# declare-lab/tango

Measured on NVIDIA H100. Metric: audio_seconds_per_second, higher is better.
Workload: dtype bf16

## Files before the change

tango_b200/csrc/gemm_tc.cu:

```cuda
#include "tng_ptx.cuh"
#include "tng_internal.h"
#include <stdlib.h>

namespace tng {

constexpr int BM = 128;
constexpr int BK = 64;
constexpr int A_TILE_BYTES = BM * BK * 2;
constexpr int GEMM_THREADS = 384;
constexpr int EPI_WARPS = 8;
constexpr int ES = 4;

struct KGroupDev {
  int view, a_c0, dw, dh, b_k0, nkb;
};

struct GemmKernelParams {
  int W, H, NB;
  int bw, bh, bn;
  int tiles_w, tiles_h, tiles_n;
  int m_tiles, n_tiles;
  int Ncols;
  int n_groups, total_kiters;
  int ksplit;
// ... 301 lines not shown
    const bool col_ok = col < p.Ncols;
    float4 add4 = make_float4(0.f, 0.f, 0.f, 0.f);
    if (col_ok && sp == 0 && p.bias) add4 = __ldg(reinterpret_cast<const float4*>(p.bias + col));
#pragma unroll 1
    for (int i = 0; i < ES; ++i) {
      const int rr = wr + 4 * i + rsub;
      if (!col_ok || rr >= nvalid) continue;
      const long long row = row_base + rr;
      float4 a = *reinterpret_cast<const float4*>(st + (4 * i + rsub) * 32 + ((cg ^ ((4 * i + rsub) & 7)) << 2));
      if (sp == 0) {
        a.x += add4.x; a.y += add4.y; a.z += add4.z; a.w += add4.w;
        if (p.rowvec) {
          const float4 r4 = __ldg(reinterpret_cast<const float4*>(p.rowvec + static_cast<long long>(n0 + rr / rpi) * p.rowvec_ld + col));
          a.x += r4.x; a.y += r4.y; a.z += r4.z; a.w += r4.w;
        }
        if (p.res) {
          if (p.res_bf16) {
            const float4 r4 = load_bf16x4(reinterpret_cast<const __nv_bfloat16*>(p.res) + row * p.ldr + col);
            a.x += r4.x; a.y += r4.y; a.z += r4.z; a.w += r4.w;
          } else {
            const float4 r4 = *reinterpret_cast<const float4*>(reinterpret_cast<const float*>(p.res) + row * p.ldr + col);
            a.x += r4.x; a.y += r4.y; a.z += r4.z; a.w += r4.w;
          }
        }
      }
      a.x *= p.alpha; a.y *= p.alpha; a.z *= p.alpha; a.w *= p.alpha;
      float* op = p.out_f32 + row * p.ld_f32 + col;
      atomicAdd(op, a.x); atomicAdd(op + 1, a.y); atomicAdd(op + 2, a.z); atomicAdd(op + 3, a.w);
    }
  }
}

template <int BN, bool FULL, bool SPLIT, bool TANH>
__device__ __forceinline__ void epi_tile_geglu(const GemmKernelParams& p, float* st, const float (&acc)[BN / 2], long long r0,
                                               int nleft, int tn, int lane) {
  constexpr int HALF = BN / 2;
  const int cg = lane & 7, rsub = lane >> 3;
#pragma unroll 1
  for (int c = 0; c < HALF / 32; ++c) {
    float4 hid[ES], g[ES];
    stage_chunk<BN>(st, lane, acc, c);
#pragma unroll
    for (int i = 0; i < ES; ++i) {
      const int r = 4 * i + rsub;
      hid[i] = *reinterpret_cast<const float4*>(st + r * 32 + ((cg ^ (r & 7)) << 2));
    }
    stage_chunk<BN>(st, lane, acc, c + HALF / 32);
#pragma unroll
    for (int i = 0; i < ES; ++i) {
      const int r = 4 * i + rsub;
      g[i] = *reinterpret_cast<const float4*>(st + r * 32 + ((cg ^ (r & 7)) << 2));
    }
    const int gcol = tn * BN + 32 * c + 4 * cg;
    const int ocol = tn * HALF + 32 * c + 4 * cg;
    float4 bh = make_float4(0.f, 0.f, 0.f, 0.f), bg = bh;
    if (p.bias) {
      bh = __ldg(reinterpret_cast<const float4*>(p.bias + gcol));
      bg = __ldg(reinterpret_cast<const float4*>(p.bias + gcol + HALF));
    }
#pragma unroll
    for (int i = 0; i < ES; ++i) {
      hid[i].x = (hid[i].x + bh.x) * (TANH ? gelu_tanh_f(g[i].x + bg.x) : gelu_erf_f(g[i].x + bg.x));
      hid[i].y = (hid[i].y + bh.y) * (TANH ? gelu_tanh_f(g[i].y + bg.y) : gelu_erf_f(g[i].y + bg.y));
      hid[i].z = (hid[i].z + bh.z) * (TANH ? gelu_tanh_f(g[i].z + bg.z) : gelu_erf_f(g[i].z + bg.z));
      hid[i].w = (hid[i].w + bh.w) * (TANH ? gelu_tanh_f(g[i].w + bg.w) : gelu_erf_f(g[i].w + bg.w));
    }
    __nv_bfloat16* op = p.out_bf16 + r0 * p.ld_bf16 + ocol;
    const long long os = 4 * p.ld_bf16;
#pragma unroll
    for (int i = 0; i < ES; ++i) {
      if (!FULL && 4 * i >= nleft) continue;
      uint2 u;
      u.x = pack_bf16(hid[i].x, hid[i].y); u.y = pack_bf16(hid[i].z, hid[i].w);
      *reinterpret_cast<uint2*>(op + i * os) = u;
      if (SPLIT) {
        uint2 l;
        l.x = pack_bf16_lo(hid[i].x, hid[i].y); l.y = pack_bf16_lo(hid[i].z, hid[i].w);
        *reinterpret_cast<uint2*>(op + p.split_off + i * os) = l;
      }
    }
  }
}

__device__ __forceinline__ int tile_kiters(const GemmKernelParams& p, int tile) {
  const int sp = tile % p.ksplit;
  return (sp + 1) * p.total_kiters / p.ksplit - sp * p.total_kiters / p.ksplit;
}

template <int BN>
__global__ void __launch_bounds__(GEMM_THREADS, 1)
gemm_tc_kernel(const __grid_constant__ CUtensorMap amap0, const __grid_constant__ CUtensorMap amap1,
               const __grid_constant__ CUtensorMap amap2, const __grid_constant__ CUtensorMap amap3,
               const __grid_constant__ CUtensorMap bmap, const __grid_constant__ GemmKernelParams p) {
  using Cfg = GemmCfg<BN>;
  constexpr int STAGES = Cfg::STAGES;
  extern __shared__ __align__(1024) uint8_t smem[];
  uint8_t* sA = smem;
  uint8_t* sB = smem + STAGES * A_TILE_BYTES;
  float* sEpi = reinterpret_cast<float*>(smem + STAGES * Cfg::STAGE_BYTES);
  uint64_t* full_bar = reinterpret_cast<uint64_t*>(smem + STAGES * Cfg::STAGE_BYTES + Cfg::EPI_BYTES);
  uint64_t* empty_bar = full_bar + STAGES;

  const int tid = threadIdx.x;
  const int warp = tid >> 5;
  const int lane = tid & 31;
  const int wg = warp >> 2;

  if (tid == 0) {
    if ((smem_u32(smem) & 1023u) != 0) __trap();
    tma_prefetch_desc(&amap0);
    tma_prefetch_desc(&bmap);
    for (int s = 0; s < STAGES; ++s) {
      mbar_init(&full_bar[s], 1);
      mbar_init(&empty_bar[s], 2);
    }
    fence_mbar_init();
  }
  __syncthreads();

  const int total_tiles = p.m_tiles * p.n_tiles * p.ksplit;
  const int work0 = blockIdx.x, work_stride = gridDim.x;

  if (wg == 0) {
    setmaxnreg_dec<40>();
    if (tid == 0) {
      uint32_t n_loaded = 0;
      for (int tile = work0; tile < total_tiles; tile += work_stride) {
        const int sp = tile % p.ksplit, t2 = tile / p.ksplit;
        const int tm = t2 / p.n_tiles, tn = t2 % p.n_tiles;
        const int tw = tm % p.tiles_w;
        const int th = (tm / p.tiles_w) % p.tiles_h;
        const int tb = tm / (p.tiles_w * p.tiles_h);
        const int w0 = tw * p.bw, h0 = th * p.bh, n0 = tb * p.bn;
        const int nk = tile_kiters(p, tile);
        int k = sp * p.total_kiters / p.ksplit, gi = 0;
        while (k >= p.g[gi].nkb) { k -= p.g[gi].nkb; ++gi; }
        for (int ki = 0; ki < nk; ++ki, ++k, ++n_loaded) {
          if (k == p.g[gi].nkb) { k = 0; ++gi; }
          const int slot = static_cast<int>(n_loaded % STAGES);
          const uint32_t use = n_loaded / STAGES;
          if (use > 0) mbar_wait(&empty_bar[slot], (use - 1) & 1);
          const KGroupDev g = p.g[gi];
          const CUtensorMap* am = g.view == 0 ? &amap0 : g.view == 1 ? &amap1 : g.view == 2 ? &amap2 : &amap3;
          mbar_arrive_expect_tx(&full_bar[slot], Cfg::STAGE_BYTES);
          tma_load_4d(sA + slot * A_TILE_BYTES, am, &full_bar[slot], g.a_c0 + k * BK, w0 + g.dw, h0 + g.dh, n0);
          tma_load_2d(sB + slot * Cfg::B_TILE_BYTES, &bmap, &full_bar[slot], g.b_k0 + k * BK, tn * BN);
        }
      }
    }
    return;
  }
  setmaxnreg_inc<232>();

  const int cw = warp - 4;
  float* st = sEpi + cw * (16 * 32);
  const int rsub = lane >> 3;
  const int wr = 16 * cw;
  const uint32_t a_off = static_cast<uint32_t>(wg - 1) * (64 * 128);
  const bool release = (tid & 127) == 0;
  const int mode = (p.res ? 1 : 0) | (p.out_f32 ? 2 : 0) | (p.out_bf16 ? 4 : 0);
  const bool geglu = (p.act == TNG_ACT_GEGLU || p.act == TNG_ACT_GEGLU_TANH);
  uint32_t n_used = 0;
  float acc[BN / 2];
#pragma unroll
  for (int i = 0; i < BN / 2; ++i) acc[i] = 0.f;
  for (int tile = work0; tile < total_tiles; tile += work_stride) {
    const int sp = tile % p.ksplit, t2 = tile / p.ksplit;
    const int tm = t2 / p.n_tiles, tn = t2 % p.n_tiles;
    const int nk = tile_kiters(p, tile);
    for (int ki = 0; ki < nk; ++ki) {
      const int slot = static_cast<int>(n_used % STAGES);
      mbar_wait(&full_bar[slot], (n_used / STAGES) & 1);
      const uint64_t ad = wgmma_desc_sw128(smem_u32(sA + slot * A_TILE_BYTES) + a_off, 16, 1024);
      const uint64_t bd = wgmma_desc_sw128(smem_u32(sB + slot * Cfg::B_TILE_BYTES), 16, 1024);
      fence_regs(acc);
      wgmma_fence();
#pragma unroll
      for (int k = 0; k < BK / 16; ++k) wgmma_ss<BN>(acc, ad + 2 * k, bd + 2 * k, (ki > 0 || k > 0) ? 1u : 0u);
      wgmma_commit();
      fence_regs(acc);
      if (ki > 0) {
        wgmma_wait<1>();
        fence_regs(acc);
        mbar_arrive_if(&empty_bar[(n_used - 1) % STAGES], release);
      }
      ++n_used;
    }
    wgmma_wait<0>();
    fence_regs(acc);
    mbar_arrive_if(&empty_bar[(n_used - 1) % STAGES], release);

    const int tw = tm % p.tiles_w;
    const int th = (tm / p.tiles_w) % p.tiles_h;
    const int tb = tm / (p.tiles_w * p.tiles_h);
    const int w0 = tw * p.bw, h0 = th * p.bh, n0 = tb * p.bn;
    const long long row_base = (static_cast<long long>(n0) * p.H + h0) * p.W + w0;
    int nvalid;
    if (p.bh == 1 && p.bn == 1) nvalid = min(BM, p.W - w0);
    else if (p.bn == 1) nvalid = min(p.bh, p.H - h0) * p.bw;
    else nvalid = min(p.bn, p.NB - n0) * p.bh * p.bw;
    const int rpi = p.bw * p.bh;
    const bool full = p.fast_epi && (nvalid == BM) && ((tn + 1) * BN <= p.Ncols);
    if (p.ksplit > 1) {
      epi_tile_splitk<BN>(p, st, acc, row_base, n0, rpi, nvalid, sp, tn, lane, wr);
    } else if (geglu) {
      if constexpr (BN == 128 || BN == 256) {
        const long long gr0 = row_base + wr + rsub;
        const int nleft = nvalid - (wr + rsub);
        if (p.act == TNG_ACT_GEGLU_TANH) {
          if (p.split_off > 0) epi_tile_geglu<BN, false, true, true>(p, st, acc, gr0, nleft, tn, lane);
          else epi_tile_geglu<BN, false, false, true>(p, st, acc, gr0, nleft, tn, lane);
        } else if (p.split_off > 0) epi_tile_geglu<BN, false, true, false>(p, st, acc, gr0, nleft, tn, lane);
        else if (nvalid == BM) epi_tile_geglu<BN, true, false, false>(p, st, acc, gr0, nleft, tn, lane);
        else epi_tile_geglu<BN, false, false, false>(p, st, acc, gr0, nleft, tn, lane);
      }
    } else if (!full) {
      EpiRows R;
      R.valid = 0;
#pragma unroll
      for (int i = 0; i < ES; ++i) {
        const int rr = wr + 4 * i + rsub;
        R.img[i] = n0 + rr / rpi;
        R.row[i] = row_base + rr;
        if (rr < nvalid) R.valid |= 1u << i;
      }
      if (p.fast_epi) epi_tile_generic<BN, true>(p, st, acc, R, tn, lane);
      else epi_tile_generic<BN, false>(p, st, acc, R, tn, lane);
    } else {
      const long long r0 = row_base + wr + rsub;
      const int img0 = n0 + (wr + rsub) / rpi;
      const bool rv_uniform = (rpi % 16) == 0;
      const long long simg = p.col_stats ? (row_base + wr) / p.stats_hw : 0;
      switch (mode) {
        case 2: epi_tile_full<BN, false, true, false>(p, st, acc, r0, img0, rv_uniform, tn, lane, simg); break;
        case 3: epi_tile_full<BN, true, true, false>(p, st, acc, r0, img0, rv_uniform, tn, lane, simg); break;
        case 4: epi_tile_full<BN, false, false, true>(p, st, acc, r0, img0, rv_uniform, tn, lane, simg); break;
        case 5: epi_tile_full<BN, true, false, true>(p, st, acc, r0, img0, rv_uniform, tn, lane, simg); break;
        case 6: epi_tile_full<BN, false, true, true>(p, st, acc, r0, img0, rv_uniform, tn, lane, simg); break;
        default: epi_tile_full<BN, true, true, true>(p, st, acc, r0, img0, rv_uniform, tn, lane, simg); break;
      }
    }
  }
}

template <int BN>
static int launch_gemm(const CUtensorMap* am, const CUtensorMap& bm, const GemmKernelParams& p, cudaStream_t st) {
  using Cfg = GemmCfg<BN>;
  const int rc = set_max_dynamic_smem<gemm_tc_kernel<BN>>(Cfg::SMEM_BYTES, "gemm_tc");
  if (rc) return rc;
  const int work = p.m_tiles * p.n_tiles * p.ksplit;
  const int grid = work < num_sms() ? work : num_sms();
  gemm_tc_kernel<BN><<<grid, GEMM_THREADS, Cfg::SMEM_BYTES, st>>>(am[0], am[1], am[2], am[3], bm, p);
  return check_launch("gemm_tc");
}

static bool is_pow2(long long x) { return x > 0 && (x & (x - 1)) == 0; }

}

using namespace tng;

static int plan_gemm(const tng_gemm_desc* d, GemmKernelParams& p, int& bn_tile_out, bool& stats_after_out) {
  if (!d) return set_error(TNG_EINVAL, "null desc");
  if (d->n_aviews < 1 || d->n_aviews > TNG_MAX_AVIEWS) return set_error(TNG_EINVAL, "n_aviews=%d", d->n_aviews);
  if (d->n_groups < 1 || d->n_groups > TNG_MAX_KGROUPS) return set_error(TNG_EINVAL, "n_groups=%d", d->n_groups);
  if (d->W <= 0 || d->H <= 0 || d->NB <= 0 || d->Ncols <= 0) return set_error(TNG_EINVAL, "bad output grid");
  if ((d->ldb > 0 ? d->ldb : d->Ktot) % 8 != 0)
    return set_error(TNG_EINVAL, "B row stride must be a multiple of 8 elements (Ktot=%lld ldb=%lld)", (long long)d->Ktot, (long long)d->ldb);

  memset(&p, 0, sizeof(p));
  p.W = d->W; p.H = d->H; p.NB = d->NB;
  if (d->W >= BM || d->H == 1) {
    p.bw = BM; p.bh = 1; p.bn = 1;
  } else {
    if (!is_pow2(d->W)) return set_error(TNG_EINVAL, "W=%d < 128 must be a power of two", d->W);
    p.bw = d->W;
    const int rem = BM / p.bw;
    if (d->H >= rem) {
      p.bh = rem; p.bn = 1;
    } else {
      if (!is_pow2(d->H)) return set_error(TNG_EINVAL, "H=%d (W=%d) must be a power of two when W*H < 128", d->H, d->W);
      p.bh = d->H; p.bn = rem / p.bh;
    }
  }
  p.tiles_w = (d->W + p.bw - 1) / p.bw;
  p.tiles_h = (d->H + p.bh - 1) / p.bh;
  p.tiles_n = (d->NB + p.bn - 1) / p.bn;
  p.m_tiles = p.tiles_w * p.tiles_h * p.tiles_n;
  p.Ncols = (int)d->Ncols;

  int bn_tile = d->block_n;
  int ksplit = 1;
  if (d->act == TNG_ACT_GEGLU || d->act == TNG_ACT_GEGLU_TANH) {
    if (bn_tile == 0) bn_tile = (d->Ncols % 256 == 0) ? 256 : 128;
    if ((bn_tile != 128 && bn_tile != 256) || d->Ncols % bn_tile != 0 || !d->out_bf16 || d->out_f32 || d->res ||
        d->rowvec)
      return set_error(TNG_EINVAL, "GEGLU epilogue needs block_n 128/256 dividing Ncols, bf16 output only");
  }
  if (bn_tile == 0) {
    const long long N = d->Ncols;
    if (N <= 32) bn_tile = 32;
    else if (N <= 64) bn_tile = 64;
    else if (N % 256 == 0 && (long long)p.m_tiles * (N / 256) >= 2 * num_sms()) bn_tile = 256;
    else if (N % 160 == 0) {
      bn_tile = 160;
      if ((long long)p.m_tiles * (N / 160) * 2 <= num_sms()) {
        static int splitk = -1;
        if (splitk < 0) { const char* e = getenv("TNG_GEMM_SPLITK"); splitk = e ? atoi(e) : 1; }
        long long kit = 0;
        for (int i = 0; i < d->n_groups; ++i) kit += d->g[i].nkb;
        const bool can_split = splitk && d->out_f32 && !d->out_bf16 && !d->accumulate && d->act == TNG_ACT_NONE &&
                               d->res != d->out_f32 && kit >= 32 && d->Ncols % 4 == 0;
        if (can_split) ksplit = 2;
        else if (N % 128 == 0 && (long long)p.m_tiles * (N / 128) <= num_sms()) bn_tile = 128;
      }
    }
    else if (N % 128 == 0) bn_tile = 128;
    else if (N % 64 == 0 && N < 256) bn_tile = 64;
    else bn_tile = 128;
  }
  p.n_tiles = (int)((d->Ncols + bn_tile - 1) / bn_tile);
  p.ksplit = ksplit;

  p.n_groups = d->n_groups;
  p.total_kiters = 0;
  for (int i = 0; i < d->n_groups; ++i) {
    const tng_kgroup& g = d->g[i];
    if (g.view < 0 || g.view >= d->n_aviews || g.nkb <= 0) return set_error(TNG_EINVAL, "k-group %d invalid", i);
    if (g.b_k0 < 0 || g.b_k0 + (long long)(g.nkb - 1) * BK >= d->Ktot)
      return set_error(TNG_EINVAL, "k-group %d: K block outside B", i);
    if (g.a_c0 < 0 || g.a_c0 + (long long)(g.nkb - 1) * BK >= d->a[g.view].C)
      return set_error(TNG_EINVAL, "k-group %d: K block outside view channels", i);
    p.g[i] = KGroupDev{g.view, g.a_c0, g.dw, g.dh, g.b_k0, g.nkb};
    p.total_kiters += g.nkb;
  }
  p.bias = d->bias; p.rowvec = d->rowvec; p.rowvec_ld = d->rowvec_ld > 0 ? d->rowvec_ld : d->Ncols; p.res = d->res; p.res_bf16 = (d->res_dtype == TNG_DT_BF16);
  p.ldr = d->ldr; p.alpha = d->alpha; p.accumulate = d->accumulate;
  p.out_f32 = d->out_f32; p.ld_f32 = d->ld_f32;
  p.out_bf16 = reinterpret_cast<__nv_bfloat16*>(d->out_bf16); p.ld_bf16 = d->ld_bf16;
  p.act = d->act; p.act_param = d->act_param; p.split_off = d->split_off;
  if (!d->out_f32 && !d->out_bf16) return set_error(TNG_EINVAL, "no output");
  if (d->accumulate && !d->out_f32) return set_error(TNG_EINVAL, "accumulate needs out_f32");

  auto al16 = [](const void* q) { return (reinterpret_cast<uintptr_t>(q) & 15) == 0; };
  bool vec = true;
  if (d->bias && !al16(d->bias)) vec = false;
  if (d->rowvec && (!al16(d->rowvec) || p.rowvec_ld % 4)) vec = false;
  if (d->res) {
    if (!al16(d->res)) vec = false;
    if (p.res_bf16 ? (d->ldr % 8) : (d->ldr % 4)) vec = false;
  }
  if (d->out_f32 && (!al16(d->out_f32) || d->ld_f32 % 4)) vec = false;
  if (d->out_bf16 && (!al16(d->out_bf16) || d->ld_bf16 % 8 || d->split_off % 8)) vec = false;
  p.vec_ok = vec ? 1 : 0;
  p.fast_epi = (vec && d->Ncols % 4 == 0) ? 1 : 0;
  if ((d->act == TNG_ACT_GEGLU || d->act == TNG_ACT_GEGLU_TANH) && !vec) return set_error(TNG_EINVAL, "GEGLU epilogue needs 16-byte aligned output");
  if (d->gn_stats) {
    if (d->stats_hw <= 0 || (static_cast<long long>(d->W) * d->H * d->NB) % d->stats_hw != 0)
      return set_error(TNG_EINVAL, "gn_stats: the output rows must be whole images of stats_hw pixels");
    if (!d->out_f32 && (d->split_off > 0 || d->act != TNG_ACT_NONE))
      return set_error(TNG_EINVAL, "gn_stats without an fp32 output needs a plain bf16 output (no activation, no hi/lo split)");
  }

  const bool full_m = (p.bh == 1 && p.bn == 1) ? (d->W % BM == 0) : (p.bn == 1 ? (d->H % p.bh == 0) : (d->NB % p.bn == 0));
  if (p.ksplit > 1 && !p.fast_epi) p.ksplit = 1;
  bool stats_after = false;
  if (d->gn_stats) {
    const bool fused = full_m && (d->Ncols % bn_tile == 0) && p.fast_epi && p.ksplit == 1 && !d->accumulate &&
                       (d->stats_hw % 16 == 0) && d->act != TNG_ACT_GEGLU && d->act != TNG_ACT_GEGLU_TANH;
    if (fused) { p.col_stats = d->gn_stats; p.stats_hw = d->stats_hw; }
    else stats_after = true;
  }
  bn_tile_out = bn_tile;
  stats_after_out = stats_after;
  return TNG_OK;
}

extern "C" int tng_gemm_plan(const tng_gemm_desc* d, int32_t* block_n, int32_t* mode, int32_t* ksplit) {
  GemmKernelParams p;
  int bn_tile = 0;
  bool stats_after = false;
  const int rc = plan_gemm(d, p, bn_tile, stats_after);
  if (rc != TNG_OK) return rc;
  if (block_n) *block_n = bn_tile;
  if (mode) *mode = 1;
  if (ksplit) *ksplit = p.ksplit;
  return TNG_OK;
}

extern "C" int tng_conv_gemm(const tng_gemm_desc* d, void* stream) {
  GemmKernelParams p;
  int bn_tile = 0;
  bool stats_after = false;
  {
    const int rc = plan_gemm(d, p, bn_tile, stats_after);
    if (rc != TNG_OK) return rc;
  }
  CUtensorMap am[4];
  for (int i = 0; i < 4; ++i) {
    const tng_aview& v = d->a[i < d->n_aviews ? i : 0];
    if (v.C % 8 != 0) return set_error(TNG_EINVAL, "view %d: C=%lld must be a multiple of 8", i, (long long)v.C);
    uint64_t dims[4] = {(uint64_t)v.C, (uint64_t)v.W, (uint64_t)v.H, (uint64_t)v.NB};
    uint64_t strides[3] = {(uint64_t)v.s_w * 2, (uint64_t)v.s_h * 2, (uint64_t)v.s_n * 2};
    uint32_t box[4] = {(uint32_t)BK, (uint32_t)p.bw, (uint32_t)p.bh, (uint32_t)p.bn};
    int rc = encode_tmap_bf16(&am[i], v.ptr, 4, dims, strides, box);
    if (rc) return rc;
  }
  CUtensorMap bm;
  {
    uint64_t dims[2] = {(uint64_t)d->Ktot, (uint64_t)d->Ncols};
    uint64_t strides[1] = {(uint64_t)(d->ldb > 0 ? d->ldb : d->Ktot) * 2};
    uint32_t box[2] = {(uint32_t)BK, (uint32_t)bn_tile};
    int rc = encode_tmap_bf16(&bm, d->b, 2, dims, strides, box);
    if (rc) return rc;
  }
  cudaStream_t st = reinterpret_cast<cudaStream_t>(stream);
  if (p.ksplit > 1) {
    const size_t rows = static_cast<size_t>(d->W) * d->H * d->NB;
    cudaError_t e = cudaMemset2DAsync(d->out_f32, static_cast<size_t>(d->ld_f32) * 4, 0, static_cast<size_t>(d->Ncols) * 4, rows, st);
    if (e != cudaSuccess) return set_error(TNG_ECUDA, "cudaMemset2DAsync(split-K output): %s", cudaGetErrorString(e));
  }
  int rc;
  switch (bn_tile) {
    case 32: rc = launch_gemm<32>(am, bm, p, st); break;
    case 64: rc = launch_gemm<64>(am, bm, p, st); break;
    case 128: rc = launch_gemm<128>(am, bm, p, st); break;
    case 160: rc = launch_gemm<160>(am, bm, p, st); break;
    case 256: rc = launch_gemm<256>(am, bm, p, st); break;
    default: return set_error(TNG_EINVAL, "block_n=%d unsupported", bn_tile);
  }
  if (rc == TNG_OK && stats_after) {
    const long long rows = static_cast<long long>(d->W) * d->H * d->NB;
    if (d->out_f32) rc = launch_col_stats(d->out_f32, TNG_DT_F32, d->Ncols, d->ld_f32, rows / d->stats_hw, d->stats_hw, d->gn_stats, st);
    else rc = launch_col_stats(d->out_bf16, TNG_DT_BF16, d->Ncols, d->ld_bf16, rows / d->stats_hw, d->stats_hw, d->gn_stats, st);
  }
  return rc;
}
```

tango_b200/csrc/tng_ptx.cuh:

```cuda
#pragma once
#include <cuda_runtime.h>
#include <cuda_bf16.h>
#include <cuda.h>
#include <stdint.h>
#include <stdio.h>
#include "../../include/tango_b200.h"

namespace tng {

#ifndef TNG_SPIN_LIMIT
#define TNG_SPIN_LIMIT (1u << 28)
#endif

__device__ __forceinline__ uint32_t smem_u32(const void* p) {
  return static_cast<uint32_t>(__cvta_generic_to_shared(p));
}

__device__ __forceinline__ void mbar_init(uint64_t* bar, uint32_t count) {
  asm volatile("mbarrier.init.shared::cta.b64 [%0], %1;" ::"r"(smem_u32(bar)), "r"(count));
}
__device__ __forceinline__ void fence_mbar_init() {
  asm volatile("fence.mbarrier_init.release.cluster;" ::: "memory");
}
__device__ __forceinline__ void mbar_arrive_expect_tx(uint64_t* bar, uint32_t bytes) {
  asm volatile("mbarrier.arrive.expect_tx.shared::cta.b64 _, [%0], %1;" ::"r"(smem_u32(bar)), "r"(bytes)
               : "memory");
}
__device__ __forceinline__ void mbar_arrive(uint64_t* bar) {
  asm volatile("mbarrier.arrive.shared::cta.b64 _, [%0];" ::"r"(smem_u32(bar)) : "memory");
}
__device__ __forceinline__ void mbar_arrive_if(uint64_t* bar, bool pred) {
  asm volatile(
      "{\n\t.reg .pred p;\n\tsetp.ne.b32 p, %1, 0;\n\t@p mbarrier.arrive.shared::cta.b64 _, [%0];\n\t}"
      ::"r"(smem_u32(bar)), "r"((uint32_t)pred) : "memory");
}
template <int N>
__device__ __forceinline__ void setmaxnreg_dec() { asm volatile("setmaxnreg.dec.sync.aligned.u32 %0;" ::"n"(N)); }
template <int N>
__device__ __forceinline__ void setmaxnreg_inc() { asm volatile("setmaxnreg.inc.sync.aligned.u32 %0;" ::"n"(N)); }
__device__ __forceinline__ uint32_t mbar_try_wait(uint64_t* bar, uint32_t parity) {
  uint32_t ok;
  asm volatile(
      "{\n\t"
      ".reg .pred P;\n\t"
      "mbarrier.try_wait.parity.shared::cta.b64 P, [%1], %2;\n\t"
      "selp.u32 %0, 1, 0, P;\n\t"
      "}\n"
      : "=r"(ok)
      : "r"(smem_u32(bar)), "r"(parity)
      : "memory");
  return ok;
}
__device__ __forceinline__ void mbar_wait(uint64_t* bar, uint32_t parity) {
  uint32_t spins = 0;
  while (!mbar_try_wait(bar, parity)) {
    if (++spins > TNG_SPIN_LIMIT) __trap();
  }
}

__device__ __forceinline__ void tma_prefetch_desc(const CUtensorMap* m) {
  asm volatile("prefetch.tensormap [%0];" ::"l"(reinterpret_cast<uint64_t>(m)) : "memory");
}
__device__ __forceinline__ void tma_load_2d(void* smem, const CUtensorMap* m, uint64_t* bar, int c0, int c1) {
  asm volatile(
      "cp.async.bulk.tensor.2d.shared::cluster.global.mbarrier::complete_tx::bytes [%0], [%1, {%3, %4}], [%2];"
      ::"r"(smem_u32(smem)), "l"(reinterpret_cast<uint64_t>(m)), "r"(smem_u32(bar)), "r"(c0), "r"(c1)
      : "memory");
}
__device__ __forceinline__ void tma_load_3d(void* smem, const CUtensorMap* m, uint64_t* bar, int c0, int c1,
                                            int c2) {
  asm volatile(
      "cp.async.bulk.tensor.3d.shared::cluster.global.mbarrier::complete_tx::bytes [%0], [%1, {%3, %4, %5}], [%2];"
      ::"r"(smem_u32(smem)), "l"(reinterpret_cast<uint64_t>(m)), "r"(smem_u32(bar)), "r"(c0), "r"(c1), "r"(c2)
      : "memory");
}
__device__ __forceinline__ void tma_load_4d(void* smem, const CUtensorMap* m, uint64_t* bar, int c0, int c1,
                                            int c2, int c3) {
  asm volatile(
      "cp.async.bulk.tensor.4d.shared::cluster.global.mbarrier::complete_tx::bytes [%0], [%1, {%3, %4, %5, %6}], "
      "[%2];" ::"r"(smem_u32(smem)),
      "l"(reinterpret_cast<uint64_t>(m)), "r"(smem_u32(bar)), "r"(c0), "r"(c1), "r"(c2), "r"(c3)
      : "memory");
}

__device__ __forceinline__ void wgmma_fence() { asm volatile("wgmma.fence.sync.aligned;" ::: "memory"); }
__device__ __forceinline__ void wgmma_commit() { asm volatile("wgmma.commit_group.sync.aligned;" ::: "memory"); }
template <int N>
__device__ __forceinline__ void wgmma_wait() {
  asm volatile("wgmma.wait_group.sync.aligned %0;" ::"n"(N) : "memory");
}
template <int R>
__device__ __forceinline__ void fence_regs(float (&d)[R]) {
#pragma unroll
  for (int i = 0; i < R; ++i) asm volatile("" : "+f"(d[i])::"memory");
}

__device__ __forceinline__ uint64_t wgmma_desc_sw128(uint32_t saddr, uint32_t lbo_bytes, uint32_t sbo_bytes) {
  uint64_t d = 0;
  d |= static_cast<uint64_t>((saddr & 0x3FFFF) >> 4);
  d |= static_cast<uint64_t>((lbo_bytes >> 4) & 0x3FFF) << 16;
  d |= static_cast<uint64_t>((sbo_bytes >> 4) & 0x3FFF) << 32;
  d |= static_cast<uint64_t>(1) << 62;
  return d;
}

template <int N>
__device__ __forceinline__ void wgmma_ss(float (&d)[N / 2], uint64_t a_desc, uint64_t b_desc, uint32_t scale_d);

template <>
__device__ __forceinline__ void wgmma_ss<32>(float (&d)[16], uint64_t a_desc, uint64_t b_desc, uint32_t scale_d) {
  asm volatile(
      "{\n\t.reg .pred p;\n\tsetp.ne.b32 p, %18, 0;\n\t"
      "wgmma.mma_async.sync.aligned.m64n32k16.f32.bf16.bf16 {%0, %1, %2, %3, %4, %5, %6, %7, %8, %9, %10, %11, %12, %13, %14, %15}, %16, %17, p, 1, 1, 0, 0;\n\t}\n"
      : "+f"(d[0]), "+f"(d[1]), "+f"(d[2]), "+f"(d[3]), "+f"(d[4]), "+f"(d[5]), "+f"(d[6]), "+f"(d[7]),
        "+f"(d[8]), "+f"(d[9]), "+f"(d[10]), "+f"(d[11]), "+f"(d[12]), "+f"(d[13]), "+f"(d[14]), "+f"(d[15])
      : "l"(a_desc), "l"(b_desc), "r"(scale_d));
}

template <>
__device__ __forceinline__ void wgmma_ss<64>(float (&d)[32], uint64_t a_desc, uint64_t b_desc, uint32_t scale_d) {
  asm volatile(
      "{\n\t.reg .pred p;\n\tsetp.ne.b32 p, %34, 0;\n\t"
      "wgmma.mma_async.sync.aligned.m64n64k16.f32.bf16.bf16 {%0, %1, %2, %3, %4, %5, %6, %7, %8, %9, %10, %11, %12, %13, %14, %15, %16, %17, %18, %19, %20, %21, %22, %23, %24, %25, %26, %27, %28, %29, %30, %31}, %32, %33, p, 1, 1, 0, 0;\n\t}\n"
      : "+f"(d[0]), "+f"(d[1]), "+f"(d[2]), "+f"(d[3]), "+f"(d[4]), "+f"(d[5]), "+f"(d[6]), "+f"(d[7]),
        "+f"(d[8]), "+f"(d[9]), "+f"(d[10]), "+f"(d[11]), "+f"(d[12]), "+f"(d[13]), "+f"(d[14]), "+f"(d[15]),
        "+f"(d[16]), "+f"(d[17]), "+f"(d[18]), "+f"(d[19]), "+f"(d[20]), "+f"(d[21]), "+f"(d[22]), "+f"(d[23]),
        "+f"(d[24]), "+f"(d[25]), "+f"(d[26]), "+f"(d[27]), "+f"(d[28]), "+f"(d[29]), "+f"(d[30]), "+f"(d[31])
      : "l"(a_desc), "l"(b_desc), "r"(scale_d));
}

template <>
__device__ __forceinline__ void wgmma_ss<128>(float (&d)[64], uint64_t a_desc, uint64_t b_desc, uint32_t scale_d) {
  asm volatile(
      "{\n\t.reg .pred p;\n\tsetp.ne.b32 p, %66, 0;\n\t"
      "wgmma.mma_async.sync.aligned.m64n128k16.f32.bf16.bf16 {%0, %1, %2, %3, %4, %5, %6, %7, %8, %9, %10, %11, %12, %13, %14, %15, %16, %17, %18, %19, %20, %21, %22, %23, %24, %25, %26, %27, %28, %29, %30, %31, %32, %33, %34, %35, %36, %37, %38, %39, %40, %41, %42, %43, %44, %45, %46, %47, %48, %49, %50, %51, %52, %53, %54, %55, %56, %57, %58, %59, %60, %61, %62, %63}, %64, %65, p, 1, 1, 0, 0;\n\t}\n"
      : "+f"(d[0]), "+f"(d[1]), "+f"(d[2]), "+f"(d[3]), "+f"(d[4]), "+f"(d[5]), "+f"(d[6]), "+f"(d[7]),
        "+f"(d[8]), "+f"(d[9]), "+f"(d[10]), "+f"(d[11]), "+f"(d[12]), "+f"(d[13]), "+f"(d[14]), "+f"(d[15]),
        "+f"(d[16]), "+f"(d[17]), "+f"(d[18]), "+f"(d[19]), "+f"(d[20]), "+f"(d[21]), "+f"(d[22]), "+f"(d[23]),
        "+f"(d[24]), "+f"(d[25]), "+f"(d[26]), "+f"(d[27]), "+f"(d[28]), "+f"(d[29]), "+f"(d[30]), "+f"(d[31]),
        "+f"(d[32]), "+f"(d[33]), "+f"(d[34]), "+f"(d[35]), "+f"(d[36]), "+f"(d[37]), "+f"(d[38]), "+f"(d[39]),
        "+f"(d[40]), "+f"(d[41]), "+f"(d[42]), "+f"(d[43]), "+f"(d[44]), "+f"(d[45]), "+f"(d[46]), "+f"(d[47]),
        "+f"(d[48]), "+f"(d[49]), "+f"(d[50]), "+f"(d[51]), "+f"(d[52]), "+f"(d[53]), "+f"(d[54]), "+f"(d[55]),
        "+f"(d[56]), "+f"(d[57]), "+f"(d[58]), "+f"(d[59]), "+f"(d[60]), "+f"(d[61]), "+f"(d[62]), "+f"(d[63])
      : "l"(a_desc), "l"(b_desc), "r"(scale_d));
}

template <>
__device__ __forceinline__ void wgmma_ss<160>(float (&d)[80], uint64_t a_desc, uint64_t b_desc, uint32_t scale_d) {
  asm volatile(
// ... 188 lines not shown
```

tango_b200/lib.py:

```python
from __future__ import annotations

import ctypes as C
import os
from typing import Optional, Sequence

import torch

from . import build as _build

ACT_NONE, ACT_SILU, ACT_LRELU, ACT_GEGLU, ACT_GEGLU_TANH = 0, 1, 2, 3, 4
DT_F32, DT_BF16 = 0, 1
MAX_AVIEWS, MAX_KGROUPS = 4, 40

SYMBOLS = [
    "tng_version", "tng_last_error", "tng_launch_count", "tng_conv_gemm", "tng_attention",
    "tng_groupnorm_stats", "tng_groupnorm_apply", "tng_layernorm", "tng_cast_act", "tng_softmax_rows",
    "tng_transpose_bf16", "tng_sched_step", "tng_timestep_embedding", "tng_linear_f32", "tng_convt_gather",
    "tng_tanh_to_i16", "tng_rmsnorm", "tng_gather_rows", "tng_rel_attention", "tng_stft_frames", "tng_stft_magnitude",
    "tng_log_clamp", "tng_attention_wide", "tng_gemm_plan",
]


class TangoB200Error(RuntimeError):
    pass
# ... 151 lines not shown

def _dt(t: torch.Tensor) -> int:
    if t.dtype == torch.float32:
        return DT_F32
    if t.dtype == torch.bfloat16:
        return DT_BF16
    raise TangoB200Error(f"unsupported dtype {t.dtype}")


def require_cuda(*ts: Optional[torch.Tensor]) -> None:
    for t in ts:
        if t is not None and not t.is_cuda:
            raise TangoB200Error("tango_b200 kernels need CUDA tensors (there is no CPU fallback)")


def require_cuda_device(device) -> None:
    if torch.device(device).type != "cuda":
        raise TangoB200Error("tango_b200 runs on CUDA only: call .to('cuda') (there is no CPU fallback)")


class View:

    __slots__ = ("t", "C", "W", "H", "NB", "s_w", "s_h", "s_n", "off")

    def __init__(self, t: torch.Tensor, C_: int, W: int, H: int, NB: int, s_w: int, s_h: int, s_n: int, off: int = 0):
        self.t, self.C, self.W, self.H, self.NB = t, C_, W, H, NB
        self.s_w, self.s_h, self.s_n, self.off = s_w, s_h, s_n, off

    @staticmethod
    def rows(t: torch.Tensor, NB: int, H: int, W: int, C_: Optional[int] = None) -> "View":
        ld = t.shape[-1]
        return View(t, ld if C_ is None else C_, W, H, NB, ld, W * ld, H * W * ld)


def conv_gemm(views: Sequence[View], groups: Sequence[tuple], weight: torch.Tensor, W: int, H: int, NB: int, *,
              bias=None, rowvec=None, res=None, alpha: float = 1.0, accumulate: bool = False, out_f32=None,
              out_bf16=None, act: int = ACT_NONE, act_param: float = 0.0, split_off: int = 0, block_n: int = 0,
              ld_f32: Optional[int] = None, ld_bf16: Optional[int] = None, ldr: Optional[int] = None,
              rowvec_ld: int = 0, algo_k: Optional[int] = None, gn_stats: Optional[torch.Tensor] = None,
              stats_hw: int = 0) -> None:
    lib = load()
    d = GemmDesc()
    require_cuda(weight, bias, rowvec, res, out_f32, out_bf16)
    assert weight.dtype == torch.bfloat16 and weight.stride(1) == 1
    d.n_aviews = len(views)
    for i, v in enumerate(views):
        require_cuda(v.t)
        assert v.t.dtype == torch.bfloat16
        d.a[i] = AView(v.t.data_ptr() + 2 * v.off, v.C, v.W, v.H, v.NB, v.s_w, v.s_h, v.s_n)
    d.b = weight.data_ptr()
    d.Ncols, d.Ktot = weight.shape
    d.ldb = weight.stride(0)
    d.W, d.H, d.NB = W, H, NB
    d.n_groups = len(groups)
    if len(groups) > MAX_KGROUPS:
        raise TangoB200Error(f"{len(groups)} k-groups > {MAX_KGROUPS}")
    for i, g in enumerate(groups):
        d.g[i] = KGroup(*g)
    d.bias = ptr(bias)
    d.rowvec = ptr(rowvec)
    d.rowvec_ld = rowvec_ld
    d.res = ptr(res)
    if res is not None:
        d.res_dtype = _dt(res)
        d.ldr = res.stride(0) if ldr is None else ldr
    d.alpha = alpha
    d.accumulate = int(accumulate)
    d.out_f32 = ptr(out_f32)
    if out_f32 is not None:
        d.ld_f32 = out_f32.stride(0) if ld_f32 is None else ld_f32
    d.out_bf16 = ptr(out_bf16)
    if out_bf16 is not None:
        d.ld_bf16 = out_bf16.stride(0) if ld_bf16 is None else ld_bf16
    d.act, d.act_param, d.split_off, d.block_n = act, act_param, split_off, block_n
    if gn_stats is not None:
        require_cuda(gn_stats)
        assert gn_stats.dtype == torch.float64 and gn_stats.is_contiguous() and stats_hw > 0
        d.gn_stats, d.stats_hw = gn_stats.data_ptr(), stats_hw
    if PROF.enabled:
        k_alg = algo_k if algo_k is not None else sum(g[5] for g in groups) * 64
        flops = 2.0 * W * H * NB * weight.shape[0] * k_alg
        bn, mode, ks = C.c_int32(0), C.c_int32(0), C.c_int32(0)
        check(lib.tng_gemm_plan(C.byref(d), C.byref(bn), C.byref(mode), C.byref(ks)), "tng_gemm_plan")
        fam = f"gemm_tc<{bn.value}" + (",splitk>" if ks.value > 1 else ">")
        PROF.timed(fam, flops, 0, lambda: check(lib.tng_conv_gemm(C.byref(d), stream_ptr()), "tng_conv_gemm"))
        return
    check(lib.tng_conv_gemm(C.byref(d), stream_ptr()), "tng_conv_gemm")


def attention(q, k, v, out, *, batch, heads, Lq, Lk, scale, q_col0=0, k_col0=0, v_col0=0, kbias=None, nsplit=1,
              q_lo_off=0, k_lo_off=0, v_lo_off=0, split_off=0) -> None:
    lib = load()
    require_cuda(q, k, v, out, kbias)
    d = AttnDesc()
    d.q, d.ld_q, d.q_col0, d.q_lo_off = q.data_ptr(), q.stride(0), q_col0, q_lo_off
    d.k, d.ld_k, d.k_col0, d.k_lo_off = k.data_ptr(), k.stride(0), k_col0, k_lo_off
    d.v, d.ld_v, d.v_col0, d.v_lo_off = v.data_ptr(), v.stride(0), v_col0, v_lo_off
    d.kbias = ptr(kbias)
    d.out, d.ld_o, d.split_off = out.data_ptr(), out.stride(0), split_off
    d.batch, d.heads, d.Lq, d.Lk, d.scale, d.nsplit = batch, heads, Lq, Lk, scale, nsplit
    PROF.timed("attention_tc", 4.0 * batch * heads * Lq * Lk * 64, 0,
               lambda: check(lib.tng_attention(C.byref(d), stream_ptr()), "tng_attention"))


def attention_wide(q, k, v, out, *, batch, L, dim, scale, q_col0=0, k_col0=0, v_col0=0) -> None:
    require_cuda(q, k, v, out)
    PROF.timed("attention_wide", 4.0 * batch * L * L * dim, 0,
               lambda: check(load().tng_attention_wide(q.data_ptr(), q.stride(0), q_col0, k.data_ptr(), k.stride(0), k_col0,
                                                       v.data_ptr(), v.stride(0), v_col0, out.data_ptr(), out.stride(0),
                                                       batch, L, dim, scale, stream_ptr()), "tng_attention_wide"))


def groupnorm_stats(x, NB, HW, stats):
    require_cuda(x, stats)
    Cc = x.shape[-1]
    _call("gn_stats", NB * HW * Cc * _esz(x), load().tng_groupnorm_stats, x.data_ptr(), _dt(x), Cc, x.stride(0), NB, HW,
          stats.data_ptr(), stream_ptr())


def groupnorm(x0, st0, x1, st1, NB, HW, groups, gamma, beta, eps, act, y, *, split_off=0, raw=None, raw_split_off=0):
    lib = load()
    require_cuda(x0, x1, st0, st1, gamma, beta, y, raw)
    C0 = x0.shape[-1]
    C1 = 0 if x1 is None else x1.shape[-1]
    rows = NB * HW
    in_bytes = rows * (C0 * _esz(x0) + C1 * _esz(x1))
    out_bytes = rows * (C0 + C1) * 2 * (2 if split_off else 1) * (2 if raw is not None else 1)
    _call("gn_apply", in_bytes + out_bytes, lib.tng_groupnorm_apply, x0.data_ptr(), _dt(x0), C0, st0.data_ptr(), ptr(x1),
          0 if x1 is None else _dt(x1), C1, ptr(st1), NB, HW, groups, gamma.data_ptr(), beta.data_ptr(), eps, act,
          y.data_ptr(), y.stride(0), split_off, ptr(raw), 0 if raw is None else raw.stride(0), raw_split_off, stream_ptr())


def layernorm(x, gamma, beta, eps, y, *, split_off=0):
    require_cuda(x, gamma, beta, y)
    rows, Cc = x.shape
    _call("layernorm", rows * Cc * (4 + (4 if split_off else 2)), load().tng_layernorm, x.data_ptr(), rows, Cc,
          gamma.data_ptr(), beta.data_ptr(), eps, y.data_ptr(), y.stride(0), split_off, stream_ptr())


def rmsnorm(x, gamma, eps, y=None, *, split_off=0, y_f32=None):
    require_cuda(x, gamma)
    rows, Cc = x.shape
    check(load().tng_rmsnorm(x.data_ptr(), rows, Cc, gamma.data_ptr(), eps, y.data_ptr() if y is not None else None,
                             y.stride(0) if y is not None else 0, split_off,
                             y_f32.data_ptr() if y_f32 is not None else None, stream_ptr()), "tng_rmsnorm")


def gather_rows(table, ids, out):
    require_cuda(table, ids, out)
    if ids.dtype != torch.int64 or not ids.is_contiguous():
        raise TangoB200Error("gather_rows: ids must be a contiguous int64 tensor")
    check(load().tng_gather_rows(table.data_ptr(), table.shape[0], ids.data_ptr(), ids.numel(), table.shape[1],
                                 out.data_ptr(), stream_ptr()), "tng_gather_rows")


def rel_attention(qkv, relbias, kbias, out, *, batch, heads, L, q_col0, k_col0, v_col0, split_off=0):
    require_cuda(qkv, relbias, out)
    check(load().tng_rel_attention(qkv.data_ptr(), qkv.stride(0), q_col0, k_col0, v_col0, batch, heads, L,
                                   relbias.data_ptr(), kbias.data_ptr() if kbias is not None else None,
                                   out.data_ptr(), out.stride(0), split_off, stream_ptr()), "tng_rel_attention")


def cast_act(x, NB, H, W, y, *, Cc=None, upsample2x=False, act=ACT_NONE, act_param=0.0, split_off=0):
    require_cuda(x, y)
    Cc = x.shape[-1] if Cc is None else Cc
    n_out = NB * H * W * (4 if upsample2x else 1) * Cc
    _call("cast_act", NB * H * W * Cc * 4 + n_out * (4 if split_off else 2), load().tng_cast_act, x.data_ptr(), NB, H,
# ... 72 lines not shown
```

Baseline: 12.17.

## Pair M-tiles in 2-CTA clusters and multicast shared B tiles via TMA

Launches the conv GEMM as 2-CTA clusters that work on adjacent M tiles with the same N tile. Each CTA loads half of the B (weight) tile and multicasts it to both CTAs, which halves global/L2 traffic for B. Empty barriers now count arrivals from both CTAs. The producer drains outstanding stages before exiting so the peer CTA is never written to after it has gone. This applies only for non-split-K plans with an even M-tile count, BN ≥ 64 and enough K iterations. The cost is a cluster scheduling constraint and extra cross-CTA synchronisation.

```diff
diff --git a/tango_b200/csrc/gemm_tc.cu b/tango_b200/csrc/gemm_tc.cu
--- a/tango_b200/csrc/gemm_tc.cu
+++ b/tango_b200/csrc/gemm_tc.cu
@@ -407,16 +407,20 @@
   }
 }
 
+template <int CL>
+__device__ __forceinline__ uint32_t cta_rank() { return CL == 2 ? cluster_ctarank() : 0u; }
+
 __device__ __forceinline__ int tile_kiters(const GemmKernelParams& p, int tile) {
   const int sp = tile % p.ksplit;
   return (sp + 1) * p.total_kiters / p.ksplit - sp * p.total_kiters / p.ksplit;
 }
 
-template <int BN>
+template <int BN, int CL>
 __global__ void __launch_bounds__(GEMM_THREADS, 1)
 gemm_tc_kernel(const __grid_constant__ CUtensorMap amap0, const __grid_constant__ CUtensorMap amap1,
                const __grid_constant__ CUtensorMap amap2, const __grid_constant__ CUtensorMap amap3,
                const __grid_constant__ CUtensorMap bmap, const __grid_constant__ GemmKernelParams p) {
+  static_assert(CL == 1 || (CL == 2 && (BN / 2) % 8 == 0), "a B half must be whole 8-row SWIZZLE_128B atoms");
   using Cfg = GemmCfg<BN>;
   constexpr int STAGES = Cfg::STAGES;
   extern __shared__ __align__(1024) uint8_t smem[];
@@ -437,22 +441,24 @@
     tma_prefetch_desc(&bmap);
     for (int s = 0; s < STAGES; ++s) {
       mbar_init(&full_bar[s], 1);
-      mbar_init(&empty_bar[s], 2);
+      mbar_init(&empty_bar[s], 2 * CL);
     }
     fence_mbar_init();
   }
-  __syncthreads();
-
-  const int total_tiles = p.m_tiles * p.n_tiles * p.ksplit;
-  const int work0 = blockIdx.x, work_stride = gridDim.x;
+  if constexpr (CL == 2) cluster_sync();
+  else __syncthreads();
+
+  const int total_tiles = (p.m_tiles / CL) * p.n_tiles * p.ksplit;
+  const int work0 = blockIdx.x / CL, work_stride = gridDim.x / CL;
 
   if (wg == 0) {
     setmaxnreg_dec<40>();
     if (tid == 0) {
+      const uint32_t crank = cta_rank<CL>();
       uint32_t n_loaded = 0;
       for (int tile = work0; tile < total_tiles; tile += work_stride) {
         const int sp = tile % p.ksplit, t2 = tile / p.ksplit;
-        const int tm = t2 / p.n_tiles, tn = t2 % p.n_tiles;
+        const int tm = (t2 / p.n_tiles) * CL + crank, tn = t2 % p.n_tiles;
         const int tw = tm % p.tiles_w;
         const int th = (tm / p.tiles_w) % p.tiles_h;
         const int tb = tm / (p.tiles_w * p.tiles_h);
@@ -469,8 +475,17 @@
           const CUtensorMap* am = g.view == 0 ? &amap0 : g.view == 1 ? &amap1 : g.view == 2 ? &amap2 : &amap3;
           mbar_arrive_expect_tx(&full_bar[slot], Cfg::STAGE_BYTES);
           tma_load_4d(sA + slot * A_TILE_BYTES, am, &full_bar[slot], g.a_c0 + k * BK, w0 + g.dw, h0 + g.dh, n0);
-          tma_load_2d(sB + slot * Cfg::B_TILE_BYTES, &bmap, &full_bar[slot], g.b_k0 + k * BK, tn * BN);
+          if constexpr (CL == 1) {
+            tma_load_2d(sB + slot * Cfg::B_TILE_BYTES, &bmap, &full_bar[slot], g.b_k0 + k * BK, tn * BN);
+          } else {
+            tma_load_2d_multicast(sB + slot * Cfg::B_TILE_BYTES + crank * (BN / 2) * 128, &bmap, &full_bar[slot],
+                                  g.b_k0 + k * BK, tn * BN + crank * (BN / 2), 0x3);
+          }
         }
+      }
+      if constexpr (CL == 2) {
+        for (uint32_t j = n_loaded; j < n_loaded + STAGES; ++j)
+          if (j >= STAGES) mbar_wait(&empty_bar[j % STAGES], (j / STAGES - 1) & 1);
       }
     }
     return;
@@ -491,7 +506,7 @@
   for (int i = 0; i < BN / 2; ++i) acc[i] = 0.f;
   for (int tile = work0; tile < total_tiles; tile += work_stride) {
     const int sp = tile % p.ksplit, t2 = tile / p.ksplit;
-    const int tm = t2 / p.n_tiles, tn = t2 % p.n_tiles;
+    const int tn = t2 % p.n_tiles;
     const int nk = tile_kiters(p, tile);
     for (int ki = 0; ki < nk; ++ki) {
       const int slot = static_cast<int>(n_used % STAGES);
@@ -508,13 +523,16 @@
         wgmma_wait<1>();
         fence_regs(acc);
         mbar_arrive_if(&empty_bar[(n_used - 1) % STAGES], release);
+        if constexpr (CL == 2) mbar_arrive_cluster_if(mapa(&empty_bar[(n_used - 1) % STAGES], cta_rank<CL>() ^ 1), release);
       }
       ++n_used;
     }
     wgmma_wait<0>();
     fence_regs(acc);
     mbar_arrive_if(&empty_bar[(n_used - 1) % STAGES], release);
-
+    if constexpr (CL == 2) mbar_arrive_cluster_if(mapa(&empty_bar[(n_used - 1) % STAGES], cta_rank<CL>() ^ 1), release);
+
+    const int tm = (t2 / p.n_tiles) * CL + cta_rank<CL>();
     const int tw = tm % p.tiles_w;
     const int th = (tm / p.tiles_w) % p.tiles_h;
     const int tb = tm / (p.tiles_w * p.tiles_h);
@@ -568,14 +586,42 @@
   }
 }
 
-template <int BN>
+template <int BN, int CL>
 static int launch_gemm(const CUtensorMap* am, const CUtensorMap& bm, const GemmKernelParams& p, cudaStream_t st) {
   using Cfg = GemmCfg<BN>;
-  const int rc = set_max_dynamic_smem<gemm_tc_kernel<BN>>(Cfg::SMEM_BYTES, "gemm_tc");
+  const int rc = set_max_dynamic_smem<gemm_tc_kernel<BN, CL>>(Cfg::SMEM_BYTES, "gemm_tc");
   if (rc) return rc;
-  const int work = p.m_tiles * p.n_tiles * p.ksplit;
-  const int grid = work < num_sms() ? work : num_sms();
-  gemm_tc_kernel<BN><<<grid, GEMM_THREADS, Cfg::SMEM_BYTES, st>>>(am[0], am[1], am[2], am[3], bm, p);
+  cudaLaunchConfig_t cfg;
+  memset(&cfg, 0, sizeof(cfg));
+  cfg.blockDim = dim3(GEMM_THREADS);
+  cfg.dynamicSmemBytes = Cfg::SMEM_BYTES;
+  cfg.stream = st;
+  cudaLaunchAttribute attr[1];
+  attr[0].id = cudaLaunchAttributeClusterDimension;
+  attr[0].val.clusterDim.x = CL;
+  attr[0].val.clusterDim.y = 1;
+  attr[0].val.clusterDim.z = 1;
+  cfg.attrs = attr;
+  cfg.numAttrs = CL > 1 ? 1 : 0;
+  static int slots = 0;
+  if (slots == 0) {
+    int n = num_sms();
+    if (CL > 1) {
+      cfg.gridDim = dim3(CL);
+      const cudaError_t e = cudaOccupancyMaxActiveClusters(&n, gemm_tc_kernel<BN, CL>, &cfg);
+      if (e != cudaSuccess || n < 1)
+        return set_error(TNG_ECUDA, "cudaOccupancyMaxActiveClusters(gemm_tc<%d,x%d>): %s (%d clusters)", BN, CL,
+                         cudaGetErrorString(e), n);
+    }
+    slots = n;
+  }
+  const int work = (p.m_tiles / CL) * p.n_tiles * p.ksplit;
+  cfg.gridDim = dim3((work < slots ? work : slots) * CL);
+  const cudaError_t e = cudaLaunchKernelEx(&cfg, gemm_tc_kernel<BN, CL>, am[0], am[1], am[2], am[3], bm, p);
+  if (e != cudaSuccess) {
+    (void)cudaGetLastError();
+    return set_error(TNG_ECUDA, "gemm_tc<%d,x%d> launch: %s", BN, CL, cudaGetErrorString(e));
+  }
   return check_launch("gemm_tc");
 }
 
@@ -585,7 +631,7 @@
 
 using namespace tng;
 
-static int plan_gemm(const tng_gemm_desc* d, GemmKernelParams& p, int& bn_tile_out, bool& stats_after_out) {
+static int plan_gemm(const tng_gemm_desc* d, GemmKernelParams& p, int& bn_tile_out, int& cl_out, bool& stats_after_out) {
   if (!d) return set_error(TNG_EINVAL, "null desc");
   if (d->n_aviews < 1 || d->n_aviews > TNG_MAX_AVIEWS) return set_error(TNG_EINVAL, "n_aviews=%d", d->n_aviews);
   if (d->n_groups < 1 || d->n_groups > TNG_MAX_KGROUPS) return set_error(TNG_EINVAL, "n_groups=%d", d->n_groups);
@@ -696,6 +742,7 @@
     if (fused) { p.col_stats = d->gn_stats; p.stats_hw = d->stats_hw; }
     else stats_after = true;
   }
+  cl_out = (p.ksplit == 1 && p.m_tiles % 2 == 0 && bn_tile >= 64 && p.total_kiters >= 10) ? 2 : 1;
   bn_tile_out = bn_tile;
   stats_after_out = stats_after;
   return TNG_OK;
@@ -703,22 +750,22 @@
 
 extern "C" int tng_gemm_plan(const tng_gemm_desc* d, int32_t* block_n, int32_t* mode, int32_t* ksplit) {
   GemmKernelParams p;
-  int bn_tile = 0;
+  int bn_tile = 0, cl = 1;
   bool stats_after = false;
-  const int rc = plan_gemm(d, p, bn_tile, stats_after);
+  const int rc = plan_gemm(d, p, bn_tile, cl, stats_after);
   if (rc != TNG_OK) return rc;
   if (block_n) *block_n = bn_tile;
-  if (mode) *mode = 1;
+  if (mode) *mode = cl;
   if (ksplit) *ksplit = p.ksplit;
   return TNG_OK;
 }
 
 extern "C" int tng_conv_gemm(const tng_gemm_desc* d, void* stream) {
   GemmKernelParams p;
-  int bn_tile = 0;
+  int bn_tile = 0, cl = 1;
   bool stats_after = false;
   {
-    const int rc = plan_gemm(d, p, bn_tile, stats_after);
+    const int rc = plan_gemm(d, p, bn_tile, cl, stats_after);
     if (rc != TNG_OK) return rc;
   }
   CUtensorMap am[4];
@@ -735,7 +782,7 @@
   {
     uint64_t dims[2] = {(uint64_t)d->Ktot, (uint64_t)d->Ncols};
     uint64_t strides[1] = {(uint64_t)(d->ldb > 0 ? d->ldb : d->Ktot) * 2};
-    uint32_t box[2] = {(uint32_t)BK, (uint32_t)bn_tile};
+    uint32_t box[2] = {(uint32_t)BK, (uint32_t)(bn_tile / cl)};
     int rc = encode_tmap_bf16(&bm, d->b, 2, dims, strides, box);
     if (rc) return rc;
   }
@@ -746,12 +793,16 @@
     if (e != cudaSuccess) return set_error(TNG_ECUDA, "cudaMemset2DAsync(split-K output): %s", cudaGetErrorString(e));
   }
   int rc;
-  switch (bn_tile) {
-    case 32: rc = launch_gemm<32>(am, bm, p, st); break;
-    case 64: rc = launch_gemm<64>(am, bm, p, st); break;
-    case 128: rc = launch_gemm<128>(am, bm, p, st); break;
-    case 160: rc = launch_gemm<160>(am, bm, p, st); break;
-    case 256: rc = launch_gemm<256>(am, bm, p, st); break;
+  switch (bn_tile * 2 + cl - 1) {
+    case 32 * 2: rc = launch_gemm<32, 1>(am, bm, p, st); break;
+    case 64 * 2: rc = launch_gemm<64, 1>(am, bm, p, st); break;
+    case 64 * 2 + 1: rc = launch_gemm<64, 2>(am, bm, p, st); break;
+    case 128 * 2: rc = launch_gemm<128, 1>(am, bm, p, st); break;
+    case 128 * 2 + 1: rc = launch_gemm<128, 2>(am, bm, p, st); break;
+    case 160 * 2: rc = launch_gemm<160, 1>(am, bm, p, st); break;
+    case 160 * 2 + 1: rc = launch_gemm<160, 2>(am, bm, p, st); break;
+    case 256 * 2: rc = launch_gemm<256, 1>(am, bm, p, st); break;
+    case 256 * 2 + 1: rc = launch_gemm<256, 2>(am, bm, p, st); break;
     default: return set_error(TNG_EINVAL, "block_n=%d unsupported", bn_tile);
   }
   if (rc == TNG_OK && stats_after) {
diff --git a/tango_b200/csrc/tng_ptx.cuh b/tango_b200/csrc/tng_ptx.cuh
--- a/tango_b200/csrc/tng_ptx.cuh
+++ b/tango_b200/csrc/tng_ptx.cuh
@@ -34,6 +34,24 @@
       "{\n\t.reg .pred p;\n\tsetp.ne.b32 p, %1, 0;\n\t@p mbarrier.arrive.shared::cta.b64 _, [%0];\n\t}"
       ::"r"(smem_u32(bar)), "r"((uint32_t)pred) : "memory");
 }
+__device__ __forceinline__ uint32_t cluster_ctarank() {
+  uint32_t r;
+  asm volatile("mov.u32 %0, %%cluster_ctarank;" : "=r"(r));
+  return r;
+}
+__device__ __forceinline__ void cluster_sync() {
+  asm volatile("barrier.cluster.arrive.release;\n\tbarrier.cluster.wait.acquire;" ::: "memory");
+}
+__device__ __forceinline__ uint32_t mapa(const void* p, uint32_t rank) {
+  uint32_t a;
+  asm volatile("mapa.shared::cluster.u32 %0, %1, %2;" : "=r"(a) : "r"(smem_u32(p)), "r"(rank));
+  return a;
+}
+__device__ __forceinline__ void mbar_arrive_cluster_if(uint32_t cluster_bar, bool pred) {
+  asm volatile(
+      "{\n\t.reg .pred p;\n\tsetp.ne.b32 p, %1, 0;\n\t@p mbarrier.arrive.shared::cluster.b64 _, [%0];\n\t}"
+      ::"r"(cluster_bar), "r"((uint32_t)pred) : "memory");
+}
 template <int N>
 __device__ __forceinline__ void setmaxnreg_dec() { asm volatile("setmaxnreg.dec.sync.aligned.u32 %0;" ::"n"(N)); }
 template <int N>
@@ -65,6 +83,14 @@
   asm volatile(
       "cp.async.bulk.tensor.2d.shared::cluster.global.mbarrier::complete_tx::bytes [%0], [%1, {%3, %4}], [%2];"
       ::"r"(smem_u32(smem)), "l"(reinterpret_cast<uint64_t>(m)), "r"(smem_u32(bar)), "r"(c0), "r"(c1)
+      : "memory");
+}
+__device__ __forceinline__ void tma_load_2d_multicast(void* smem, const CUtensorMap* m, uint64_t* bar, int c0, int c1,
+                                                      uint16_t cta_mask) {
+  asm volatile(
+      "cp.async.bulk.tensor.2d.shared::cluster.global.mbarrier::complete_tx::bytes.multicast::cluster"
+      " [%0], [%1, {%3, %4}], [%2], %5;"
+      ::"r"(smem_u32(smem)), "l"(reinterpret_cast<uint64_t>(m)), "r"(smem_u32(bar)), "r"(c0), "r"(c1), "h"(cta_mask)
       : "memory");
 }
 __device__ __forceinline__ void tma_load_3d(void* smem, const CUtensorMap* m, uint64_t* bar, int c0, int c1,
diff --git a/tango_b200/lib.py b/tango_b200/lib.py
--- a/tango_b200/lib.py
+++ b/tango_b200/lib.py
@@ -257,7 +257,7 @@
         flops = 2.0 * W * H * NB * weight.shape[0] * k_alg
         bn, mode, ks = C.c_int32(0), C.c_int32(0), C.c_int32(0)
         check(lib.tng_gemm_plan(C.byref(d), C.byref(bn), C.byref(mode), C.byref(ks)), "tng_gemm_plan")
-        fam = f"gemm_tc<{bn.value}" + (",splitk>" if ks.value > 1 else ">")
+        fam = f"gemm_tc<{bn.value}" + (",splitk>" if ks.value > 1 else ",x2>" if mode.value == 2 else ">")
         PROF.timed(fam, flops, 0, lambda: check(lib.tng_conv_gemm(C.byref(d), stream_ptr()), "tng_conv_gemm"))
         return
     check(lib.tng_conv_gemm(C.byref(d), stream_ptr()), "tng_conv_gemm")
```

Measured after the change: 12.51 (median of 6 runs). 1.03x the previous value.
